# lukemelas/deep-spectral-segmentation

Hardware: AMD Instinct MI355X
Metric: images/sec end-to-end (features+eigs) at 480², K=5; eigvec cos-err vs CPU (higher is better)
Workload: dtype f16

## Files before the change

### deep-spectral-segmentation_amd/csrc/linear384.hip

```cpp
#include "common.h"
#include "kres.h"
#include <type_traits>
#include <utility>

#ifdef DSS_LIN_TIMELINE
__device__ unsigned long long dss_lin_tl[8];
#define DSS_TL_DECL unsigned long long tl_t = __builtin_readcyclecounter(), tl_acc[4] = {0, 0, 0, 0}; const unsigned long long tl_r0 = wall_clock64();
#define DSS_TL_MARK(i) { const unsigned long long n_ = __builtin_readcyclecounter(); tl_acc[i] += n_ - tl_t; tl_t = n_; }
#define DSS_TL_FLUSH if (threadIdx.x == 0) { for (int i_ = 0; i_ < 4; ++i_) atomicAdd(&dss_lin_tl[i_], tl_acc[i_]); atomicAdd(&dss_lin_tl[4], 1ull); atomicAdd(&dss_lin_tl[5], wall_clock64() - tl_r0); }
#else
#define DSS_TL_DECL
#define DSS_TL_MARK(i)
#define DSS_TL_FLUSH
#endif

namespace dss {

static constexpr int LBN = 32;
static constexpr int LGELU_ILP = 2;

template <int OFF, class V> __device__ __forceinline__ void lds_read_b128_at(V& dst, unsigned addr) {
  asm volatile("ds_read_b128 %0, %1 offset:%2" : "=v"(dst) : "v"(addr), "n"(OFF));
}
template <int N, class V> __device__ __forceinline__ void lds_wait_for(V& v) {
  asm volatile("s_waitcnt lgkmcnt(%1)" : "+v"(v) : "n"(N));
}
template <int N> __device__ __forceinline__ void wait_vmcnt() { asm volatile("s_waitcnt vmcnt(%0)" ::"n"(N) : "memory"); }
template <int... I, class F> __device__ __forceinline__ void static_for_impl(std::integer_sequence<int, I...>, F&& f) {
  (f(std::integral_constant<int, I>{}), ...);
}
template <int N, class F> __device__ __forceinline__ void static_for(F&& f) {
  static_for_impl(std::make_integer_sequence<int, N>{}, static_cast<F&&>(f));
}

// ... 5 lines not shown
    if (RES && NUNIT > 2) { pp[1] = n; n += 4; }
    for (int v = 0; v < NUNIT; ++v) {
      if (v == u) {
        int last = px[u];
        if (RES && pp[u >> 1] > last) last = pp[u >> 1];
        return n - (last + 4);
      }
      if (ST) n += 4;
      if (v + NXS < NUNIT) { px[v + NXS] = n; n += 4; }
      if (RES && (v & 1) && (v >> 1) + 2 < NUNIT / 2) { pp[(v >> 1) + 2] = n; n += 4; }
    }
    return 0;
  }
};

template <int KS, int RT, int NW> struct LinCfg {
  static_assert(KS * RT == 48 && KS % NW == 0, "the A operand of a wave is 48 fragments");
  static constexpr int WAVES = NW, THREADS = 64 * NW;
  static constexpr int K = 16 * KS;
  static constexpr int ROWS_WAVE = 32 * RT;
  static constexpr int ROWS = ROWS_WAVE * NW;
  static constexpr int CHUNK_BYTES = LBN * K * 2;
  static constexpr int PATCH_BYTES = ROWS_WAVE * 128;
  static constexpr int MAXN = KS == 24 ? 2048 : 3072;
  static constexpr int NSTORE = 4 * RT;
};

struct KfOut { float* k32; float* rnorm; int Tn; float eps; const unsigned char* img; const float* pos; int H, W, Wp; };

template <class T, int GELU, int KS, int RT, int NW, int LNM, int MODE>
__device__ __forceinline__ void linear_kres_body(const T* __restrict__ A, float* __restrict__ X,
                                                 const T* __restrict__ R, long r_ld, long r_plane, float eps,
                                                 const T* __restrict__ W,
                                                 const T* __restrict__ bias, const float* __restrict__ aux,
                                                 T* __restrict__ C, int M, int N, int planar, const KfOut kf) {
  typedef typename vec8<T>::type V8;
  typedef typename vec4<T>::type V4;
  typedef LinCfg<KS, RT, NW> Cfg;
  constexpr int LK = Cfg::K, LKS = KS, LBM = Cfg::ROWS, LWAVES = NW, LTHREADS = Cfg::THREADS;
  __shared__ __attribute__((aligned(256))) unsigned char Ws[2][Cfg::CHUNK_BYTES];
  __shared__ __attribute__((aligned(256))) unsigned char Stg[LWAVES][Cfg::PATCH_BYTES];
  const int tid = threadIdx.x;
  const int lane = tid & 63, wave = tid >> 6;
  const int li = lane & 31, hh = lane >> 5;
  const int mrem = M - blockIdx.x * LBM;
  const int rloc = wave * Cfg::ROWS_WAVE;
  const bool block_full = mrem >= LBM;

  DSS_TL_DECL
  V8 a[RT][LKS];
  float am[RT];
  if constexpr (MODE == 4) {
    static_assert(RT == 1 && LK == 768, "one 16 x 16 x 3 patch per operand row");
    typedef unsigned u32x2v __attribute__((ext_vector_type(2)));
    const unsigned gp = (unsigned)min((int)blockIdx.x * LBM + rloc + li, M - 1);
    const unsigned pb = gp / (unsigned)kf.Tn, pn = gp - pb * (unsigned)kf.Tn;
    const unsigned py0 = (pn / (unsigned)kf.Wp) * 16u, px0 = (pn - (pn / (unsigned)kf.Wp) * (unsigned)kf.Wp) * 16u;
    const unsigned w3 = (unsigned)kf.W * 3u;
// ... 45 lines not shown
      if constexpr (rd + 1 < NROUND) wait_vmcnt<NPIECE>();
      else wait_vmcnt<0>();
      const unsigned char* pw = pbuf[rd & 1];
#pragma unroll
      for (int t = 0; t < RT; ++t)
#pragma unroll
        for (int sl = 0; sl < 4; ++sl)
          a[t][4 * rd + sl] = *reinterpret_cast<const V8*>(pw + (32 * t + li) * 128 + ((((unsigned)(2 * sl + hh)) ^ fsw) << 4));
      asm volatile("s_waitcnt lgkmcnt(0)" ::: "memory");
      if constexpr (rd + 2 < NROUND) issue_round(rd + 2);
    });
    __syncthreads();
  } else {
    typedef __attribute__((address_space(3))) void* lds3_t;
    typedef float f32x4v __attribute__((ext_vector_type(4)));
    constexpr bool RES = LNM == 2;
    constexpr int NCB = LK / 32, NUNIT = RT * NCB;
    constexpr int WS_SHARE = 2 * Cfg::CHUNK_BYTES / LWAVES;
    constexpr int NSLOT = (WS_SHARE + Cfg::PATCH_BYTES) / 4096;
    constexpr int NXS = RES ? NSLOT - 2 : NSLOT;
    static_assert(WS_SHARE % 4096 == 0 && Cfg::PATCH_BYTES % 4096 == 0 && NXS >= 2 && NCB % 2 == 0 && NUNIT <= 48, "LN prologue layout");
    constexpr bool XST = RES && MODE != 2;
    typedef LnSched<NUNIT, NXS, RES, XST> Sched;
    unsigned char* const ws_share = &Ws[0][0] + wave * WS_SHARE;
    unsigned char* const patch = &Stg[wave][0];
    auto slot_ptr = [&](int i) -> unsigned char* { return i * 4096 < WS_SHARE ? ws_share + i * 4096 : patch + (i * 4096 - WS_SHARE); };
    const size_t row0 = (size_t)blockIdx.x * LBM;
    const unsigned char* const xblk = reinterpret_cast<const unsigned char*>(X) + row0 * (size_t)(LK * 4);
    const unsigned char* const rblk = reinterpret_cast<const unsigned char*>(R) + row0 * (size_t)r_ld * 2;
    const unsigned r_ldb = (unsigned)r_ld * 2u;
    const unsigned fsw16 = 16u * (unsigned)((li >> 1) & 7);
    const int prow = lane >> 3;
    const unsigned pch16[2] = {16u * (unsigned)((lane & 7) ^ (lane >> 4)), 16u * (unsigned)((lane & 7) ^ (4 + (lane >> 4)))};
    auto dma = [&](unsigned lds_addr, unsigned voff, const unsigned char* sbase) {
      unsigned keep;
      asm volatile("s_mov_b32 %0, m0\n\ts_mov_b32 m0, %1\n\ts_nop 0\n\tglobal_load_lds_dwordx4 %2, %3\n\t"
                   "s_mov_b32 m0, %0"
                   : "=&s"(keep) : "s"(lds_addr), "v"(voff), "s"(sbase) : "memory");
// ... 6 lines not shown
    auto rowc = [&](int t, int q) { return (unsigned)min(rloc + 32 * t + 8 * q + prow, mrem - 1); };
    auto issue_x = [&](int u) {
      const int t = u / NCB, cb = u % NCB;
      const unsigned dst = __builtin_amdgcn_readfirstlane((unsigned)(size_t)(lds3_t)slot_ptr(u % NXS));
      const unsigned char* src = uniform_ptr(xblk + 128 * cb);
#pragma unroll
      for (int q = 0; q < 4; ++q) dma(dst + 1024u * q, rowc(t, q) * (unsigned)(LK * 4) + pch16[q & 1], src);
    };
    auto issue_p = [&](int j) {
      const int t = (2 * j) / NCB, g = ((2 * j) % NCB) >> 1;
      const unsigned dst = __builtin_amdgcn_readfirstlane((unsigned)(size_t)(lds3_t)slot_ptr(NXS + (j & 1)));
      const unsigned char* src = uniform_ptr(rblk + (size_t)g * (size_t)r_plane * 2);
#pragma unroll
      for (int q = 0; q < 4; ++q) dma(dst + 1024u * q, rowc(t, q) * r_ldb + pch16[q & 1], src);
    };
    float piv[RT], s1[RT], s2[RT];
#pragma unroll
    for (int t = 0; t < RT; ++t) { piv[t] = 0.f; s1[t] = 0.f; s2[t] = 0.f; }
    if (RES) issue_p(0);
#pragma unroll
    for (int i = 0; i < NXS && i < NUNIT; ++i) issue_x(i);
    if (RES && NUNIT > 2) issue_p(1);
    static_for<NUNIT>([&](auto uc) {
      constexpr int u = decltype(uc)::value;
      constexpr int t = u / NCB, cb = u % NCB, o = cb & 1;
      if (block_full) wait_vmcnt<Sched::after(u)>();
      else wait_vmcnt<0>();
      unsigned char* xs = slot_ptr(u % NXS);
      unsigned char* xr = xs + li * 128;
      f32x4v v0[2], v1[2];
#pragma unroll
      for (int sl = 0; sl < 2; ++sl) {
        v0[sl] = *reinterpret_cast<const f32x4v*>(xr + ((16u * (4 * sl + 2 * hh)) ^ fsw16));
        v1[sl] = *reinterpret_cast<const f32x4v*>(xr + ((16u * (4 * sl + 2 * hh + 1)) ^ fsw16));
      }
      if constexpr (RES) {
        const unsigned char* pr = slot_ptr(NXS + ((u >> 1) & 1)) + li * 128;
#pragma unroll
        for (int sl = 0; sl < 2; ++sl) {
          const V8 pv = *reinterpret_cast<const V8*>(pr + ((16u * (4 * o + 2 * sl + hh)) ^ fsw16));
#pragma unroll
          for (int e = 0; e < 4; ++e) { v0[sl][e] += to_f32<T>(pv[e]); v1[sl][e] += to_f32<T>(pv[4 + e]); }
        }
      }
      if constexpr (cb == 0) {
        const float g0 = __builtin_amdgcn_fmed3f(v0[0][0], v0[0][1], v0[0][2]), g1 = __builtin_amdgcn_fmed3f(v1[0][0], v1[0][1], v1[0][2]);
        const float g2 = __builtin_amdgcn_fmed3f(v0[1][0], v0[1][1], v0[1][2]);
        const unsigned pm = __float_as_uint(__builtin_amdgcn_fmed3f(g0, g1, g2));
        const auto pr = __builtin_amdgcn_permlane32_swap(pm, pm, false, false);
        const unsigned plo = pr[0];
        piv[t] = __uint_as_float(plo);
// ... 20 lines not shown
#pragma unroll
        for (int sl = 0; sl < 2; ++sl) {
          *reinterpret_cast<f32x4v*>(xr + ((16u * (4 * sl + 2 * hh)) ^ fsw16)) = v0[sl];
          *reinterpret_cast<f32x4v*>(xr + ((16u * (4 * sl + 2 * hh + 1)) ^ fsw16)) = v1[sl];
        }
        asm volatile("s_waitcnt lgkmcnt(0)" ::: "memory");
        unsigned char* xw = const_cast<unsigned char*>(xblk) + 128 * cb;
#pragma unroll
        for (int q = 0; q < 4; ++q) {
          const f32x4v lin = *reinterpret_cast<const f32x4v*>(xs + 1024 * q + 16 * lane);
          if (block_full || rloc + 32 * t + 8 * q + prow < mrem)
            *reinterpret_cast<f32x4v*>(xw + rowc(t, q) * (unsigned)(LK * 4) + pch16[q & 1]) = lin;
        }
      }
      asm volatile("s_waitcnt lgkmcnt(0)" ::: "memory");
      if (u + NXS < NUNIT) issue_x(u + NXS);
      if (RES && (u & 1) && (u >> 1) + 2 < NUNIT / 2) issue_p((u >> 1) + 2);
    });
    constexpr float HN = (float)(LK / 2);
#pragma unroll
    for (int t = 0; t < RT; ++t) {
      const float mh = piv[t] + s1[t] * (1.0f / HN), m2h = fmaxf(s2[t] - s1[t] * s1[t] * (1.0f / HN), 0.f);
      const float mo = __shfl_xor(mh, 32, 64), m2o = __shfl_xor(m2h, 32, 64);
      const float mean = 0.5f * (mh + mo), dl = mo - mh;
      const float var = (m2h + m2o + dl * dl * (0.5f * HN)) * (1.0f / (float)LK);
      am[t] = hh ? (var + eps) * rsqrtf(var + eps) : mean - piv[t];
    }
    __syncthreads();
  }

  constexpr int NST = LKS / LWAVES;
  const unsigned gsrc0 = (unsigned)(li * (LK * 2) + 16 * hh + 32 * (wave * NST));
// ... 283 lines not shown
    DSS_TL_MARK(3)
  }
  if constexpr (MODE == 2) kf_finish();
  DSS_TL_FLUSH
}

template <class T, int GELU, int KS, int RT, int NW, int LNM, int MODE = 0>
__global__ __launch_bounds__(64 * NW, NW == 8 ? 1 : 2) void linear_kres_kernel(const T* __restrict__ A, float* __restrict__ X,
                                                                 const T* __restrict__ R, long r_ld, long r_plane, float eps,
                                                                 const T* __restrict__ W,
                                                                 const T* __restrict__ bias, const float* __restrict__ aux,
                                                                 T* __restrict__ C, int M, int N, int planar) {
  linear_kres_body<T, GELU, KS, RT, NW, LNM, MODE>(A, X, R, r_ld, r_plane, eps, W, bias, aux, C, M, N, planar, KfOut{nullptr, nullptr, 0, 0.f, nullptr, nullptr, 0, 0, 0});
}

template <class T>
__global__ __launch_bounds__(512, 1) void patch_embed_kres_kernel(const unsigned char* __restrict__ img, const T* __restrict__ Wp,
                                                                  const T* __restrict__ biasp, const float* __restrict__ pos,
                                                                  float* __restrict__ x, int M, int N, int Np, int H, int W, int Wpat) {
  linear_kres_body<T, 0, 48, 1, 8, 0, 4>(nullptr, nullptr, nullptr, 0, 0, 0.f, Wp, biasp, nullptr, nullptr, M, N, 0,
                                             KfOut{x, nullptr, Np, 0.f, img, pos, H, W, Wpat});
}

template <class T, int KS, int RT, int NW, int LNM>
__global__ __launch_bounds__(64 * NW, NW == 8 ? 1 : 2) void kfeat_kres_kernel(float* __restrict__ X, const T* __restrict__ R, long r_ld, long r_plane, float eps,
                                                            const T* __restrict__ W, const float* __restrict__ aux, f16* __restrict__ k16,
                                                            float* __restrict__ k32, float* __restrict__ rnorm, int M, int Tn, float norm_eps) {
  linear_kres_body<T, 0, KS, RT, NW, LNM, 2>(nullptr, X, R, r_ld, r_plane, eps, W, nullptr, aux, reinterpret_cast<T*>(k16), M, 16 * KS, 0,
                                                 KfOut{k32, rnorm, Tn, norm_eps, nullptr, nullptr, 0, 0, 0});
}
// ... 26 lines not shown
  if constexpr (std::is_same<T, f16>::value) {
    if (gelu == 2) {
      hipLaunchKernelGGL((linear_kres_kernel<T, 2, KS, RT, NW, LNM, MODE>), dim3(blocks), dim3(64 * NW), 0, s, (const T*)A, X,
                         (const T*)R, r_ld, r_plane, eps, (const T*)W, (const T*)bias, aux, (T*)C, M, N, planar);
      return;
    }
  }
  if (gelu)
    hipLaunchKernelGGL((linear_kres_kernel<T, 1, KS, RT, NW, LNM, MODE>), dim3(blocks), dim3(64 * NW), 0, s, (const T*)A, X,
                       (const T*)R, r_ld, r_plane, eps, (const T*)W, (const T*)bias, aux, (T*)C, M, N, planar);
  else
    hipLaunchKernelGGL((linear_kres_kernel<T, 0, KS, RT, NW, LNM, MODE>), dim3(blocks), dim3(64 * NW), 0, s, (const T*)A, X,
                       (const T*)R, r_ld, r_plane, eps, (const T*)W, (const T*)bias, aux, (T*)C, M, N, planar);
}

template <int KS, int RT, int NW>
static int linear_kres(const char* name, const void* A, float* X, const void* res, int res_layout, float eps, const void* W,
                       const void* bias, const float* aux, void* C, int M, int N, int gelu, int out_layout, int dtype,
                       void* stream) {
  typedef LinCfg<KS, RT, NW> Cfg;
  DSS_REQUIRE((A ? bias != nullptr : (X && aux)) && W && C, "%s: null pointer", name);
  DSS_REQUIRE(gelu == 0 || gelu == 1 || (gelu == 2 && dtype == DSS_F16), "%s: gelu must be 0, 1 (fp32 erf form) or 2 (packed-f16 form, DSS_F16 only) (got %d)", name, gelu);
  DSS_REQUIRE(M > 0 && N > 0 && N % (2 * LBN) == 0 && N <= Cfg::MAXN, "%s: need M > 0, N %% %d == 0, N <= %d (M=%d N=%d)",
              name, 2 * LBN, Cfg::MAXN, M, N);
  DSS_REQUIRE(out_layout == DSS_ROW_MAJOR || out_layout == DSS_PLANAR64,
              "%s: out_layout must be DSS_ROW_MAJOR or DSS_PLANAR64 (got %d)", name, out_layout);
  DSS_REQUIRE(A || res_layout == DSS_ROW_MAJOR || res_layout == DSS_PLANAR64,
              "%s: res_layout must be DSS_ROW_MAJOR or DSS_PLANAR64 (got %d)", name, res_layout);
  DSS_REQUIRE(A || (eps >= 0.f && (const void*)X != res && (const void*)X != C && res != C), "%s: eps < 0 or aliased buffers", name);
  hipStream_t s = (hipStream_t)stream;
  const int planar = out_layout == DSS_PLANAR64;
  const long r_ld = res_layout == DSS_PLANAR64 ? 64 : Cfg::K, r_plane = res_layout == DSS_PLANAR64 ? 64L * M : 64;
#define DSS_LAUNCH_KRES(TT)                                                                                              \
  do {                                                                                                                   \
    if (A) launch_linear_kres<TT, KS, RT, NW, 0>(A, nullptr, nullptr, 0, 0, 0.f, W, bias, nullptr, C, M, N, gelu, planar, s); \
    else if (!res) launch_linear_kres<TT, KS, RT, NW, 1>(nullptr, X, nullptr, 0, 0, eps, W, nullptr, aux, C, M, N, gelu, planar, s); \
    else launch_linear_kres<TT, KS, RT, NW, 2>(nullptr, X, res, r_ld, r_plane, eps, W, nullptr, aux, C, M, N, gelu, planar, s); \
  } while (0)
  switch (dtype) {
    case DSS_F16: DSS_LAUNCH_KRES(f16); break;
    case DSS_BF16: DSS_LAUNCH_KRES(bf16); break;
    default: return fail(DSS_ERR_BAD_ARG, "%s: dtype must be DSS_F16 or DSS_BF16 (got %d)", name, dtype);
  }
#undef DSS_LAUNCH_KRES
  DSS_CHECK_LAUNCH(name);
  return DSS_OK;
}

}

extern "C" int dss_linear_k384(const void* A, const void* W, const void* bias, void* C, int M, int N, int gelu,
// ... 19 lines not shown
      hipLaunchKernelGGL((dss::lnlinear_prepare_kernel<dss::f16>), dim3(N), dim3(64), 0, s, W, bias, gamma, beta, (dss::f16*)Wg, aux, K);
      break;
    case DSS_BF16:
      hipLaunchKernelGGL((dss::lnlinear_prepare_kernel<dss::bf16>), dim3(N), dim3(64), 0, s, W, bias, gamma, beta, (dss::bf16*)Wg, aux, K);
      break;
    default: return dss::fail(DSS_ERR_BAD_ARG, "dss_lnlinear_prepare: dtype must be DSS_F16 or DSS_BF16 (got %d)", dtype);
  }
  DSS_CHECK_LAUNCH("dss_lnlinear_prepare");
  return DSS_OK;
}

extern "C" int dss_lnlinear_k384(float* x, const void* residual, int res_layout, float eps, const void* Wg, const float* aux,
                                 void* C, int M, int N, int gelu, int out_layout, int dtype, void* stream) {
  DSS_REQUIRE(x, "dss_lnlinear_k384: null pointer");
  return dss::linear_kres<24, 2, 4>("dss_lnlinear_k384", nullptr, x, residual, res_layout, eps, Wg, nullptr, aux, C, M, N, gelu, out_layout, dtype, stream);
}

extern "C" int dss_patch_embed_p16(const uint8_t* img_u8, const void* Wp, const void* biasp, const float* pos, float* x, int B, int H, int W,
                                   int D, int dtype, void* stream) {
  DSS_REQUIRE(img_u8 && Wp && biasp && pos && x, "dss_patch_embed_p16: null pointer");
  DSS_REQUIRE(B > 0 && H >= 16 && W >= 16, "dss_patch_embed_p16: bad shape B=%d H=%d W=%d", B, H, W);
  typedef dss::LinCfg<48, 1, 8> Cfg;
  DSS_REQUIRE(D > 0 && D % (2 * dss::LBN) == 0 && D <= Cfg::MAXN, "dss_patch_embed_p16: need D %% %d == 0, D <= %d (D=%d)", 2 * dss::LBN, Cfg::MAXN, D);
  const int Hp = H / 16, Wpat = W / 16, Np = Hp * Wpat;
  const long M = (long)B * Np;
  DSS_REQUIRE(M * Np < 4294967296L && (M + B) * D * 4 < 4294967296L && (long)H * W * 3 * B < (1L << 46),
              "dss_patch_embed_p16: B=%d x %d patches exceeds the 32-bit row arithmetic of the epilogue", B, Np);
  const int blocks = dss::ceil_div((int)M, Cfg::ROWS);
  hipStream_t s = (hipStream_t)stream;
  switch (dtype) {
// ... 63 lines not shown
```

### deep-spectral-segmentation_amd/hip.py

```python
from __future__ import annotations

import ctypes
import functools
import os
from ctypes import c_char_p, c_float, c_int, c_size_t, c_uint, c_void_p
from pathlib import Path
from typing import Optional

import torch

PKG = Path(__file__).resolve().parent
LIB_PATH = PKG / "lib" / "libdss_hip.so"

DSS_F32, DSS_F16, DSS_BF16 = 0, 1, 2
_DTYPE_CODE = {torch.float32: DSS_F32, torch.float16: DSS_F16, torch.bfloat16: DSS_BF16}

SYMBOLS = {
    "dss_abi_version": (c_int, []),
    "dss_last_error": (c_char_p, []),
    "dss_target_arch": (c_char_p, []),
    "dss_preprocess_chw": (c_int, [c_void_p, c_void_p, c_int, c_int, c_int, c_void_p]),
    "dss_preprocess_patchify": (c_int, [c_void_p, c_void_p, c_int, c_int, c_int, c_int, c_int, c_void_p]),
    "dss_layernorm_fwd": (c_int, [c_void_p, c_void_p, c_int, c_int, c_void_p, c_void_p, c_void_p, c_int, c_int, c_int,
                                  c_float, c_void_p]),
    "dss_attention_fwd": (c_int, [c_void_p, c_int, c_void_p, c_int, c_int, c_int, c_float, c_int, c_void_p]),
    "dss_linear_k384": (c_int, [c_void_p, c_void_p, c_void_p, c_void_p, c_int, c_int, c_int, c_int, c_int, c_void_p]),
    "dss_linear_k768": (c_int, [c_void_p, c_void_p, c_void_p, c_void_p, c_int, c_int, c_int, c_int, c_int, c_void_p]),
    "dss_linear_lt_workspace_bytes": (c_size_t, []),
    "dss_linear_lt": (c_int, [c_void_p, c_void_p, c_void_p, c_void_p, ctypes.c_long, c_int, c_int, c_int, c_int, c_void_p, c_size_t,
                              c_void_p]),
    "dss_linear_lt_accumulate": (c_int, [c_void_p, c_void_p, c_void_p, c_void_p, ctypes.c_long, c_int, c_int, c_int, c_void_p, c_size_t,
                                         c_void_p]),
    "dss_linear_lt_describe": (c_int, [ctypes.c_long, c_int, c_int, c_int, c_int, c_int, c_size_t, c_char_p, c_size_t]),
    "dss_lnlinear_prepare": (c_int, [c_void_p, c_void_p, c_void_p, c_void_p, c_void_p, c_void_p, c_int, c_int, c_int,
                                     c_void_p]),
    "dss_lnlinear_k384": (c_int, [c_void_p, c_void_p, c_int, c_float, c_void_p, c_void_p, c_void_p, c_int, c_int, c_int,
                                  c_int, c_int, c_void_p]),
    "dss_lnlinear_k768": (c_int, [c_void_p, c_void_p, c_int, c_float, c_void_p, c_void_p, c_void_p, c_int, c_int, c_int,
                                  c_int, c_int, c_void_p]),
    "dss_lnlinear_kfeatures_k384": (c_int, [c_void_p, c_void_p, c_int, c_float, c_void_p, c_void_p, c_void_p, c_void_p,
                                            c_void_p, c_int, c_int, c_float, c_void_p]),
    "dss_lnlinear_kfeatures": (c_int, [c_void_p, c_void_p, c_int, c_float, c_void_p, c_void_p, c_void_p, c_void_p,
                                       c_void_p, c_int, c_int, c_int, c_float, c_int, c_void_p]),
    "dss_patch_embed_p16": (c_int, [c_void_p, c_void_p, c_void_p, c_void_p, c_void_p, c_int, c_int, c_int, c_int, c_int, c_void_p]),
    "dss_normalize_rows": (c_int, [c_void_p, c_void_p, c_int, c_int, c_float, c_void_p]),
    "dss_affinity_ld": (c_int, [c_int]),
    "dss_affinity_elems": (c_size_t, [c_int]),
    "dss_affinity": (c_int, [c_void_p, c_void_p, c_int, c_int, c_int, c_int, c_void_p]),
    "dss_affinity_split_workspace_bytes": (c_size_t, [c_int, c_int, c_int]),
    "dss_affinity_split": (c_int, [c_void_p, c_void_p, c_int, c_int, c_int, c_int, c_float, c_int, c_void_p, c_size_t,
                                   c_void_p]),
    "dss_affinity_split_u16": (c_int, [c_void_p, c_void_p, c_int, c_int, c_int, c_float, c_void_p, c_size_t, c_void_p]),
    "dss_affinity_fused_u16": (c_int, [c_void_p, c_void_p, c_int, c_int, c_int, c_float, c_void_p]),
    "dss_affinity_f16_u16": (c_int, [c_void_p, c_void_p, c_void_p, c_int, c_int, c_int, c_void_p]),
# ... 273 lines not shown

def lnlinear_prepare(weight: torch.Tensor, bias: torch.Tensor, gamma: torch.Tensor, beta: torch.Tensor,
                     dtype: torch.dtype):
    n, k = weight.shape
    for t in (weight, bias, gamma, beta):
        assert t.dtype == torch.float32
    wg = torch.empty((n, k), dtype=dtype, device=weight.device)
    aux = torch.empty((n, 2), dtype=torch.float32, device=weight.device)
    _check(load_library().dss_lnlinear_prepare(_dev(weight, "weight"), _dev(bias, "bias"), _dev(gamma, "gamma"),
                                               _dev(beta, "beta"), _dev(wg, "Wg"), _dev(aux, "aux"), n, k, dtype_code(dtype),
                                               _stream()), "dss_lnlinear_prepare")
    return wg, aux


def lnlinear(x: torch.Tensor, residual: Optional[torch.Tensor], wg: torch.Tensor, aux: torch.Tensor, eps: float,
             gelu: bool = False, planar: bool = False, residual_planar: bool = False) -> torch.Tensor:
    assert x.dtype == torch.float32 and aux.dtype == torch.float32
    k = x.shape[-1]
    if k not in LINEAR_KRES_WIDTHS:
        raise ValueError(f"lnlinear: reduction dimension must be one of {sorted(LINEAR_KRES_WIDTHS)} (got {k})")
    n = wg.shape[0]
    m = x.numel() // k
    assert wg.shape[1] == k and tuple(aux.shape) == (n, 2)
    if residual is not None:
        assert residual.dtype == wg.dtype and tuple(residual.shape) == ((k // 64, m, 64) if residual_planar else tuple(x.shape))
    entry = LINEAR_KRES_WIDTHS[k][0].replace("dss_linear", "dss_lnlinear")
    shape = (n // 64, m, 64) if planar else (*x.shape[:-1], n)
    out = torch.empty(shape, dtype=wg.dtype, device=x.device)
    with _timed("lnlinear", m=m, n=n, k=k, gelu=gelu, res=residual is not None):
        _check(getattr(load_library(), entry)(_dev(x, "x"), 0 if residual is None else _dev(residual, "residual"),
                                              PLANAR64 if residual_planar else ROW_MAJOR, float(eps), _dev(wg, "Wg"),
                                              _dev(aux, "aux"), _dev(out, "out"), m, n, int(gelu),
                                              PLANAR64 if planar else ROW_MAJOR, dtype_code(wg.dtype), _stream()), entry)
    return out


def lnlinear_kfeatures(x: torch.Tensor, residual: Optional[torch.Tensor], wg: torch.Tensor, aux: torch.Tensor, eps: float,
                       norm_eps: float = 1e-12, residual_planar: bool = False, out=None):
    assert x.dtype == torch.float32 and x.dim() == 3 and x.shape[-1] in (384, 768) and x.is_contiguous()
    b, t, d = x.shape
    assert wg.dtype in (torch.float16, torch.bfloat16) and tuple(wg.shape) == (d, d) and tuple(aux.shape) == (d, 2)
    if t <= 64:
        raise ValueError(f"lnlinear_kfeatures: needs more than 64 tokens per image (got {t})")
    if residual is not None:
        assert residual.dtype == wg.dtype and tuple(residual.shape) == ((d // 64, b * t, 64) if residual_planar else (b, t, d))
    if out is not None:
        k32, k16, rn = out
# ... 224 lines not shown
```

### deep-spectral-segmentation_amd/vit.py

```python
from __future__ import annotations

import math
from pathlib import Path
from typing import Dict, Optional, Tuple

import torch
import torch.nn.functional as F

from . import hip
from .synthetic import VIT_CONFIGS

LN_EPS = 1e-6
_TUNING_FILE = Path(__file__).resolve().parent / "tuning" / "tunableop_gfx950.csv"
_gemm_tuning_ready = False


def setup_gemm_tuning(tune_new_shapes: bool = False, use_table: bool = True) -> None:
    global _gemm_tuning_ready
    if not use_table:
        return
    tun = torch.cuda.tunable
    if not _gemm_tuning_ready:
        tun.enable(True)
        if hasattr(tun, "write_file_on_exit"):
# ... 17 lines not shown
    dim = pos_embed.shape[-1]
    side = int(math.sqrt(n0))
    grid = pos_embed[:, 1:].reshape(1, side, side, dim).permute(0, 3, 1, 2)
    grid = F.interpolate(grid, scale_factor=((hp + 0.1) / side, (wp + 0.1) / side), mode="bicubic")
    if (grid.shape[-2], grid.shape[-1]) != (hp, wp):
        raise RuntimeError(f"pos-embed interpolation produced {tuple(grid.shape[-2:])}, wanted {(hp, wp)}")
    grid = grid.permute(0, 2, 3, 1).reshape(1, -1, dim)
    return torch.cat((pos_embed[:, :1], grid), dim=1)


class DinoViT:

    def __init__(self, model_name: str, state_dict: Dict[str, torch.Tensor], device: torch.device,
                 dtype: torch.dtype = torch.float16, k_proj_fp32: bool = False, gelu: str = "auto",
                 linear_kres: int = 2, fuse_ln: bool = True, gemm_tuning: str = "table", fuse_k: bool = True, fuse_pe: bool = True,
                 fuse_qkv768: bool = True, library_gemm: str = "lt", fc2_into_stream: bool = False):
        name = model_name.lower()
        if name not in VIT_CONFIGS:
            raise ValueError(f"Cannot get model: {model_name}")
        if dtype not in (torch.float16, torch.bfloat16):
            raise ValueError("compute dtype must be torch.float16 or torch.bfloat16")
        self.model_name = name
        self.embed_dim, self.depth, self.num_heads, self.patch_size = VIT_CONFIGS[name]
        self.device, self.dtype = torch.device(device), dtype
        self.k_proj_fp32 = k_proj_fp32
        if gelu not in ("auto", "erf", "erf_f16", "tanh_fused"):
            raise ValueError("gelu must be 'auto', 'erf' (DINO's exact GELU, fp32 arithmetic), 'erf_f16' (the same function evaluated on "
                             "packed f16: f16 operands and the K-resident fc1 kernel only) or 'tanh_fused'")
        if gelu == "auto":
            gelu = "erf_f16" if self.embed_dim == 384 else "erf"
        if gelu == "erf_f16" and (dtype != torch.float16 or linear_kres < 2 or self.embed_dim not in hip.LINEAR_KRES_WIDTHS):
            gelu = "erf"
        self.gelu = gelu
        self._gelu_code = 2 if gelu == "erf_f16" else 1
        if linear_kres not in (0, 1, 2):
            raise ValueError("linear_kres must be 0, 1 or 2")
        self.linear_k384 = int(linear_kres)
        self.fuse_ln = bool(fuse_ln)
        self.fuse_k = bool(fuse_k)
        self.fuse_qkv768 = bool(fuse_qkv768)
        if library_gemm not in ("lt", "torch"):
            raise ValueError("library_gemm must be 'lt' (dss_linear_lt) or 'torch' (F.linear)")
        self.library_gemm = library_gemm
        self.fc2_into_stream = bool(fc2_into_stream) and library_gemm == "lt"
        d = self.embed_dim
        sd = state_dict
        need = ["cls_token", "pos_embed", "patch_embed.proj.weight", "patch_embed.proj.bias"]
        for i in range(self.depth):
            for s in ("norm1.weight", "norm1.bias", "attn.qkv.weight", "attn.qkv.bias", "attn.proj.weight",
                      "attn.proj.bias", "norm2.weight", "norm2.bias", "mlp.fc1.weight", "mlp.fc1.bias",
                      "mlp.fc2.weight", "mlp.fc2.bias"):
                need.append(f"blocks.{i}.{s}")
        missing = [k for k in need if k not in sd]
        if missing:
            raise KeyError(f"state_dict is missing {len(missing)} DINO ViT keys, e.g. {missing[:3]}")

        def lp(t):
            return t.detach().to(self.device, dtype).contiguous()

        def f32(t):
# ... 55 lines not shown
        k384 = bool(self.linear_k384) and d == 384
        kres_fc1 = self.gelu in ("erf", "erf_f16") and self.linear_k384 >= 2 and d in hip.LINEAR_KRES_WIDTHS
        lib = ("library GEMM (hipBLASLt through dss_linear_lt: no Stream-K split, verified)" if self.library_gemm == "lt"
               else "library GEMM (hipBLASLt through F.linear)")
        return {
            "patch_embed": "dss_patch_embed_p16 (transform + GEMM + position rows, one kernel)" if self.pe16 is not None
                           else f"dss_preprocess_patchify + {lib} + add",
            "norm1+qkv": f"dss_lnlinear_k{d}" if ("qkv_wg" in blk and self.linear_k384) else
                         ("dss_layernorm_fwd + dss_linear_k384" if k384 else f"dss_layernorm_fwd + {lib}"),
            "attention": "dss_attention_fwd",
            "proj": "dss_linear_k384" if k384 else lib,
            "norm2+fc1+gelu": f"dss_lnlinear_k{d}" if (kres_fc1 and "fc1_wg" in blk) else
                              (f"dss_layernorm_fwd + dss_linear_k{d}" if kres_fc1 else f"dss_layernorm_fwd + {lib} + GELU pass"),
            "gelu": {"erf": "exact-erf form in fp32 (A&S 7.1.28, |err| <= 3e-7)", "erf_f16": "erf-GELU polynomial form on packed f16 (csrc/kres.h)",
                     "tanh_fused": "hipBLASLt's tanh epilogue (NOT the reference function)"}[self.gelu],
            "fc2": lib + (" adding into the fp32 residual stream (dss_linear_lt_accumulate)" if self.fc2_into_stream else ""),
            "hooked norm1 + K projection + hand-over": "dss_lnlinear_kfeatures" if "k_wg" in self.blocks[-1] else
                                                       f"dss_layernorm_fwd + {lib} + dss_kfeatures_finalize",
        }

    def _pos(self, h: int, w: int) -> Tuple[torch.Tensor, torch.Tensor]:
        key = (h, w)
        if key not in self._pos_cache:
            pe = interpolate_pos_encoding(self.pos_embed, self.patch_size, h, w)
            cls_row = (self.cls_token[0, 0] + pe[0, 0]).to(self.device)
            self._pos_cache[key] = (cls_row.contiguous(), pe[0, 1:].to(self.device).contiguous())
        return self._pos_cache[key]

    @torch.no_grad()
    def _run_blocks(self, img_u8: torch.Tensor, nblocks: int):
# ... 8 lines not shown
            key = ("pe16", hp * p, wp * p)
            if key not in self._pos_cache:
                self._pos_cache[key] = (pos + self.pe16[1]).contiguous()
            hip.patch_embed16(img_u8.contiguous(), self.pe16[0], None, self._pos_cache[key], x)
        else:
            patches = hip.preprocess_patchify(img_u8.contiguous(), p, self.dtype)
            tok = self._linear(patches, self.pe_w, self.pe_b, "patch_embed")
            torch.add(tok, pos, out=x[:, 1:])

        pending = None
        k384 = self.linear_k384 and d == 384
        kres_fc1 = self.gelu in ("erf", "erf_f16") and self.linear_k384 >= 2 and d in hip.LINEAR_KRES_WIDTHS
        for i in range(nblocks):
            blk = self.blocks[i]
            qkv_planar = bool(k384)
            if "qkv_wg" in blk and self.linear_k384:
                qkv = hip.lnlinear(x, pending, blk["qkv_wg"], blk["qkv_aux"], LN_EPS, planar=True)
                qkv_planar = True
            else:
                hcur = hip.layernorm(x, blk["n1w"], blk["n1b"], LN_EPS, self.dtype, residual=pending)
                if k384:
                    qkv = hip.linear_kres(hcur, blk["qkv_w"], blk["qkv_b"], planar=True)
                else:
                    qkv = self._linear(hcur, blk["qkv_w"], blk["qkv_b"], "qkv")
            o = hip.attention(qkv, heads, self.scale, planar_bt=(b, t)) if qkv_planar else hip.attention(qkv, heads, self.scale)
            if k384:
                pending = hip.linear_kres(o, blk["proj_w"], blk["proj_b"], planar=True)
            else:
                pending = self._linear(o, blk["proj_w"], blk["proj_b"], "proj")
            if kres_fc1 and "fc1_wg" in blk:
                f1 = hip.lnlinear(x, pending, blk["fc1_wg"], blk["fc1_aux"], LN_EPS, gelu=self._gelu_code, residual_planar=bool(k384))
            else:
                hcur = hip.layernorm(x, blk["n2w"], blk["n2b"], LN_EPS, self.dtype, residual=pending,
                                     residual_planar=bool(k384))
                if kres_fc1:
                    f1 = hip.linear_kres(hcur, blk["fc1_w"], blk["fc1_b"], gelu=self._gelu_code)
                elif self.gelu in ("erf", "erf_f16"):
                    f1 = F.gelu(self._linear(hcur, blk["fc1_w"], blk["fc1_b"], "fc1"))
                else:
                    f1 = torch._addmm_activation(blk["fc1_b"], hcur.view(b * t, d), blk["fc1_w"].t(),
                                                 use_gelu=True).view(b, t, -1)
            if self.fc2_into_stream:
                hip.linear_lt_accumulate(f1, blk["fc2_w"], blk["fc2_b32"], x, what="fc2")
                pending = None
            else:
# ... 76 lines not shown
```

### include/dss_hip.h

```cpp
#ifndef DSS_HIP_H
#define DSS_HIP_H

#include <stddef.h>
#include <stdint.h>

#ifdef __cplusplus
extern "C" {
#endif

#define DSS_ABI_VERSION 10

enum { DSS_F32 = 0, DSS_F16 = 1, DSS_BF16 = 2 };

enum { DSS_ROW_MAJOR = 0, DSS_PLANAR64 = 1 };

enum {
  DSS_OK = 0,
  DSS_ERR_BAD_ARG = -1,
  DSS_ERR_HIP = -2,
  DSS_ERR_WORKSPACE = -3,
  DSS_ERR_NO_CONVERGENCE = -4
};

int dss_abi_version(void);
// ... 18 lines not shown

size_t dss_linear_lt_workspace_bytes(void);
int dss_linear_lt(const void* A, const void* W, const void* bias, void* C, long M, int N, int K, int dtype, int out_dtype,
                  void* workspace, size_t workspace_bytes, void* stream);
int dss_linear_lt_describe(long M, int N, int K, int dtype, int out_dtype, int has_bias, size_t workspace_bytes, char* buf,
                           size_t buflen);
int dss_linear_lt_accumulate(const void* A, const void* W, const float* bias, float* X, long M, int N, int K, int dtype,
                             void* workspace, size_t workspace_bytes, void* stream);

int dss_lnlinear_prepare(const float* W, const float* bias, const float* gamma, const float* beta, void* Wg, float* aux,
                         int N, int K, int dtype, void* stream);
int dss_lnlinear_k384(float* x, const void* residual, int res_layout, float eps, const void* Wg, const float* aux, void* C,
                      int M, int N, int gelu, int out_layout, int dtype, void* stream);
int dss_lnlinear_k768(float* x, const void* residual, int res_layout, float eps, const void* Wg, const float* aux, void* C,
                      int M, int N, int gelu, int out_layout, int dtype, void* stream);

int dss_lnlinear_kfeatures_k384(float* x, const void* residual, int res_layout, float eps, const void* Wg, const float* aux,
                                float* k32, void* k16, float* rnorm, int M, int T, float norm_eps, void* stream);
int dss_lnlinear_kfeatures(float* x, const void* residual, int res_layout, float eps, const void* Wg, const float* aux,
                           float* k32, void* k16, float* rnorm, int M, int T, int D, float norm_eps, int dtype, void* stream);

int dss_patch_embed_p16(const uint8_t* img_u8, const void* Wp, const void* biasp, const float* pos, float* x, int B, int H, int W,
                        int D, int dtype, void* stream);

int dss_normalize_rows(const float* x, float* y, int rows, int D, float eps, void* stream);

int dss_affinity_ld(int N);
size_t dss_affinity_elems(int N);
int dss_affinity(const float* feats, float* W, int B, int N, int D, int threshold_at_zero,
                 void* stream);
// ... 40 lines not shown
```

Measured before the change: 13860.

## Store the fp32 residual stream once per ViT block via read-only and two-residual LN-Linear

Adds a read-only LN+Linear variant for the qkv path, which normalises x plus the pending residual without writing the sum back. It also adds a two-residual variant for fc1 that adds the previous fc2 output and the attention projection output in its prologue and stores the updated stream once. The goal is to cut one fp32 read-modify-write of the residual stream per block. In exchange the fc1 prologue loads an extra f16 residual tile through a new DMA schedule, which adds LDS slot pressure and a new schedule helper.

```diff
diff --git a/deep-spectral-segmentation_amd/csrc/linear384.hip b/deep-spectral-segmentation_amd/csrc/linear384.hip
--- a/deep-spectral-segmentation_amd/csrc/linear384.hip
+++ b/deep-spectral-segmentation_amd/csrc/linear384.hip
@@ -18,6 +18,7 @@
 
 static constexpr int LBN = 32;
 static constexpr int LGELU_ILP = 2;
+static constexpr int LN2_RD = 2;
 
 template <int OFF, class V> __device__ __forceinline__ void lds_read_b128_at(V& dst, unsigned addr) {
   asm volatile("ds_read_b128 %0, %1 offset:%2" : "=v"(dst) : "v"(addr), "n"(OFF));
@@ -53,6 +54,23 @@
   }
 };
 
+template <int NUNIT, int NXS, int RD> struct LnSched2 {
+  static constexpr int after(int u) {
+    int n = 0, px[64] = {}, pp[64] = {};
+    for (int i = 0; i < NUNIT && i < (NXS > RD ? NXS : RD); ++i) {
+      if (i < RD) { n += 4; pp[i] = n; }
+      if (i < NXS) { n += 4; px[i] = n; }
+    }
+    for (int v = 0; v < NUNIT; ++v) {
+      if (v == u) return n - (px[u] > pp[u] ? px[u] : pp[u]);
+      n += 4;
+      if (v + RD < NUNIT) { n += 4; pp[v + RD] = n; }
+      if (v + NXS < NUNIT) { n += 4; px[v + NXS] = n; }
+    }
+    return 0;
+  }
+};
+
 template <int KS, int RT, int NW> struct LinCfg {
   static_assert(KS * RT == 48 && KS % NW == 0, "the A operand of a wave is 48 fragments");
   static constexpr int WAVES = NW, THREADS = 64 * NW;
@@ -72,7 +90,8 @@
                                                  const T* __restrict__ R, long r_ld, long r_plane, float eps,
                                                  const T* __restrict__ W,
                                                  const T* __restrict__ bias, const float* __restrict__ aux,
-                                                 T* __restrict__ C, int M, int N, int planar, const KfOut kf) {
+                                                 T* __restrict__ C, int M, int N, int planar, const KfOut kf,
+                                                 const T* __restrict__ R2 = nullptr, long r2_ld = 0, long r2_plane = 0) {
   typedef typename vec8<T>::type V8;
   typedef typename vec4<T>::type V4;
   typedef LinCfg<KS, RT, NW> Cfg;
@@ -80,7 +99,7 @@
   __shared__ __attribute__((aligned(256))) unsigned char Ws[2][Cfg::CHUNK_BYTES];
   __shared__ __attribute__((aligned(256))) unsigned char Stg[LWAVES][Cfg::PATCH_BYTES];
   const int tid = threadIdx.x;
-  const int lane = tid & 63, wave = tid >> 6;
+  const int lane = tid & 63, wave = LNM == 4 ? __builtin_amdgcn_readfirstlane(tid >> 6) : tid >> 6;
   const int li = lane & 31, hh = lane >> 5;
   const int mrem = M - blockIdx.x * LBM;
   const int rloc = wave * Cfg::ROWS_WAVE;
@@ -156,14 +175,16 @@
   } else {
     typedef __attribute__((address_space(3))) void* lds3_t;
     typedef float f32x4v __attribute__((ext_vector_type(4)));
-    constexpr bool RES = LNM == 2;
+    constexpr bool RES = LNM >= 2, RES2 = LNM == 4;
+    static_assert(LNM <= 2 || (KS == 24 && MODE == 0), "the read-only and two-residual prologues are built for the K = 384 Linear mode only");
     constexpr int NCB = LK / 32, NUNIT = RT * NCB;
     constexpr int WS_SHARE = 2 * Cfg::CHUNK_BYTES / LWAVES;
     constexpr int NSLOT = (WS_SHARE + Cfg::PATCH_BYTES) / 4096;
-    constexpr int NXS = RES ? NSLOT - 2 : NSLOT;
+    constexpr int RD2 = LN2_RD;
+    constexpr int NXS = RES2 ? NSLOT - RD2 : RES ? NSLOT - 2 : NSLOT;
     static_assert(WS_SHARE % 4096 == 0 && Cfg::PATCH_BYTES % 4096 == 0 && NXS >= 2 && NCB % 2 == 0 && NUNIT <= 48, "LN prologue layout");
-    constexpr bool XST = RES && MODE != 2;
-    typedef LnSched<NUNIT, NXS, RES, XST> Sched;
+    constexpr bool XST = RES && MODE != 2 && LNM != 3;
+    typedef std::conditional_t<RES2, LnSched2<NUNIT, NXS, RD2>, LnSched<NUNIT, NXS, RES, XST>> Sched;
     unsigned char* const ws_share = &Ws[0][0] + wave * WS_SHARE;
     unsigned char* const patch = &Stg[wave][0];
     auto slot_ptr = [&](int i) -> unsigned char* { return i * 4096 < WS_SHARE ? ws_share + i * 4096 : patch + (i * 4096 - WS_SHARE); };
@@ -200,13 +221,41 @@
 #pragma unroll
       for (int q = 0; q < 4; ++q) dma(dst + 1024u * q, rowc(t, q) * r_ldb + pch16[q & 1], src);
     };
+    auto rtile_ptr = [&](int s, int u) -> unsigned char* {
+      const int o = NXS * 4096 + 2048 * (s * RD2 + u % RD2);
+      return o < WS_SHARE ? ws_share + o : patch + (o - WS_SHARE);
+    };
+    auto issue_p2 = [&](int u) {
+      const int t = u / NCB, cb = u % NCB;
+      unsigned fl;
+      asm volatile("v_mbcnt_lo_u32_b32 %0, -1, 0\n\tv_mbcnt_hi_u32_b32 %0, -1, %0" : "=v"(fl));
+      const unsigned ch16 = 16u * ((fl & 3u) ^ ((fl >> 4) & 3u));
+#pragma unroll
+      for (int s = 0; s < 2; ++s) {
+        const unsigned dst = __builtin_amdgcn_readfirstlane((unsigned)(size_t)(lds3_t)rtile_ptr(s, u));
+        const unsigned char* blk2 = s ? reinterpret_cast<const unsigned char*>(R2) + row0 * (size_t)r2_ld * 2 : rblk;
+        const unsigned char* src = uniform_ptr(blk2 + (size_t)(cb >> 1) * (size_t)(s ? r2_plane : r_plane) * 2 + 64 * (cb & 1));
+        const unsigned ldb = s ? (unsigned)r2_ld * 2u : r_ldb;
+#pragma unroll
+        for (int q = 0; q < 2; ++q)
+          dma(dst + 1024u * q, (unsigned)min(rloc + 32 * t + 16 * q + (int)(fl >> 2), mrem - 1) * ldb + ch16, src);
+      }
+    };
     float piv[RT], s1[RT], s2[RT];
 #pragma unroll
     for (int t = 0; t < RT; ++t) { piv[t] = 0.f; s1[t] = 0.f; s2[t] = 0.f; }
-    if (RES) issue_p(0);
-#pragma unroll
-    for (int i = 0; i < NXS && i < NUNIT; ++i) issue_x(i);
-    if (RES && NUNIT > 2) issue_p(1);
+    if constexpr (RES2) {
+#pragma unroll
+      for (int i = 0; i < NUNIT && i < (NXS > RD2 ? NXS : RD2); ++i) {
+        if (i < RD2) issue_p2(i);
+        if (i < NXS) issue_x(i);
+      }
+    } else {
+      if (RES) issue_p(0);
+#pragma unroll
+      for (int i = 0; i < NXS && i < NUNIT; ++i) issue_x(i);
+      if (RES && NUNIT > 2) issue_p(1);
+    }
     static_for<NUNIT>([&](auto uc) {
       constexpr int u = decltype(uc)::value;
       constexpr int t = u / NCB, cb = u % NCB, o = cb & 1;
@@ -220,7 +269,19 @@
         v0[sl] = *reinterpret_cast<const f32x4v*>(xr + ((16u * (4 * sl + 2 * hh)) ^ fsw16));
         v1[sl] = *reinterpret_cast<const f32x4v*>(xr + ((16u * (4 * sl + 2 * hh + 1)) ^ fsw16));
       }
-      if constexpr (RES) {
+      if constexpr (RES2) {
+        const unsigned rsw16 = 16u * (unsigned)((li >> 2) & 3);
+#pragma unroll
+        for (int s = 0; s < 2; ++s) {
+          const unsigned char* pr = rtile_ptr(s, u) + li * 64;
+#pragma unroll
+          for (int sl = 0; sl < 2; ++sl) {
+            const V8 pv = *reinterpret_cast<const V8*>(pr + ((16u * (2 * sl + hh)) ^ rsw16));
+#pragma unroll
+            for (int e = 0; e < 4; ++e) { v0[sl][e] += to_f32<T>(pv[e]); v1[sl][e] += to_f32<T>(pv[4 + e]); }
+          }
+        }
+      } else if constexpr (RES) {
         const unsigned char* pr = slot_ptr(NXS + ((u >> 1) & 1)) + li * 128;
 #pragma unroll
         for (int sl = 0; sl < 2; ++sl) {
@@ -271,8 +332,13 @@
         }
       }
       asm volatile("s_waitcnt lgkmcnt(0)" ::: "memory");
-      if (u + NXS < NUNIT) issue_x(u + NXS);
-      if (RES && (u & 1) && (u >> 1) + 2 < NUNIT / 2) issue_p((u >> 1) + 2);
+      if constexpr (RES2) {
+        if (u + RD2 < NUNIT) issue_p2(u + RD2);
+        if (u + NXS < NUNIT) issue_x(u + NXS);
+      } else {
+        if (u + NXS < NUNIT) issue_x(u + NXS);
+        if (RES && (u & 1) && (u >> 1) + 2 < NUNIT / 2) issue_p((u >> 1) + 2);
+      }
     });
     constexpr float HN = (float)(LK / 2);
 #pragma unroll
@@ -586,6 +652,15 @@
   linear_kres_body<T, GELU, KS, RT, NW, LNM, MODE>(A, X, R, r_ld, r_plane, eps, W, bias, aux, C, M, N, planar, KfOut{nullptr, nullptr, 0, 0.f, nullptr, nullptr, 0, 0, 0});
 }
 
+template <class T, int GELU>
+__global__ __launch_bounds__(256, 2) void linear_kres2_kernel(float* __restrict__ X, const T* __restrict__ R, long r_ld, long r_plane,
+                                                              const T* __restrict__ R2, long r2_ld, long r2_plane, float eps,
+                                                              const T* __restrict__ W, const float* __restrict__ aux, T* __restrict__ C,
+                                                              int M, int N, int planar) {
+  linear_kres_body<T, GELU, 24, 2, 4, 4, 0>(nullptr, X, R, r_ld, r_plane, eps, W, nullptr, aux, C, M, N, planar,
+                                            KfOut{nullptr, nullptr, 0, 0.f, nullptr, nullptr, 0, 0, 0}, R2, r2_ld, r2_plane);
+}
+
 template <class T>
 __global__ __launch_bounds__(512, 1) void patch_embed_kres_kernel(const unsigned char* __restrict__ img, const T* __restrict__ Wp,
                                                                   const T* __restrict__ biasp, const float* __restrict__ pos,
@@ -642,11 +717,29 @@
                        (const T*)R, r_ld, r_plane, eps, (const T*)W, (const T*)bias, aux, (T*)C, M, N, planar);
 }
 
+template <class T>
+static void launch_linear_kres2(float* X, const void* R, long r_ld, long r_plane, const void* R2, long r2_ld, long r2_plane, float eps,
+                                const void* W, const float* aux, void* C, int M, int N, int gelu, int planar, hipStream_t s) {
+  const int blocks = ceil_div(M, LinCfg<24, 2, 4>::ROWS);
+#define DSS_LAUNCH_KRES2(G)                                                                                                      \
+  hipLaunchKernelGGL((linear_kres2_kernel<T, G>), dim3(blocks), dim3(256), 0, s, X, (const T*)R, r_ld, r_plane, (const T*)R2, r2_ld, \
+                     r2_plane, eps, (const T*)W, aux, (T*)C, M, N, planar)
+  if constexpr (std::is_same<T, f16>::value) {
+    if (gelu == 2) { DSS_LAUNCH_KRES2(2); return; }
+  }
+  if (gelu) DSS_LAUNCH_KRES2(1);
+  else DSS_LAUNCH_KRES2(0);
+#undef DSS_LAUNCH_KRES2
+}
+
 template <int KS, int RT, int NW>
 static int linear_kres(const char* name, const void* A, float* X, const void* res, int res_layout, float eps, const void* W,
                        const void* bias, const float* aux, void* C, int M, int N, int gelu, int out_layout, int dtype,
-                       void* stream) {
+                       void* stream, bool store = true, const void* res2 = nullptr, int res2_layout = DSS_ROW_MAJOR) {
   typedef LinCfg<KS, RT, NW> Cfg;
+  DSS_REQUIRE((store && !res2) || (KS == 24 && !A && res && (store || !res2)), "%s: the read-only and two-residual forms need K = 384 and a residual", name);
+  DSS_REQUIRE(!res2 || ((res2_layout == DSS_ROW_MAJOR || res2_layout == DSS_PLANAR64) && res2 != (const void*)X && res2 != C),
+              "%s: res2_layout must be DSS_ROW_MAJOR or DSS_PLANAR64 (got %d) and residual2 must not alias x or C", name, res2_layout);
   DSS_REQUIRE((A ? bias != nullptr : (X && aux)) && W && C, "%s: null pointer", name);
   DSS_REQUIRE(gelu == 0 || gelu == 1 || (gelu == 2 && dtype == DSS_F16), "%s: gelu must be 0, 1 (fp32 erf form) or 2 (packed-f16 form, DSS_F16 only) (got %d)", name, gelu);
   DSS_REQUIRE(M > 0 && N > 0 && N % (2 * LBN) == 0 && N <= Cfg::MAXN, "%s: need M > 0, N %% %d == 0, N <= %d (M=%d N=%d)",
@@ -659,10 +752,13 @@
   hipStream_t s = (hipStream_t)stream;
   const int planar = out_layout == DSS_PLANAR64;
   const long r_ld = res_layout == DSS_PLANAR64 ? 64 : Cfg::K, r_plane = res_layout == DSS_PLANAR64 ? 64L * M : 64;
+  const long r2_ld = res2_layout == DSS_PLANAR64 ? 64 : Cfg::K, r2_plane = res2_layout == DSS_PLANAR64 ? 64L * M : 64;
 #define DSS_LAUNCH_KRES(TT)                                                                                              \
   do {                                                                                                                   \
     if (A) launch_linear_kres<TT, KS, RT, NW, 0>(A, nullptr, nullptr, 0, 0, 0.f, W, bias, nullptr, C, M, N, gelu, planar, s); \
     else if (!res) launch_linear_kres<TT, KS, RT, NW, 1>(nullptr, X, nullptr, 0, 0, eps, W, nullptr, aux, C, M, N, gelu, planar, s); \
+    else if (KS == 24 && res2) launch_linear_kres2<TT>(X, res, r_ld, r_plane, res2, r2_ld, r2_plane, eps, W, aux, C, M, N, gelu, planar, s); \
+    else if (KS == 24 && !store) launch_linear_kres<TT, 24, 2, 4, 3>(nullptr, X, res, r_ld, r_plane, eps, W, nullptr, aux, C, M, N, gelu, planar, s); \
     else launch_linear_kres<TT, KS, RT, NW, 2>(nullptr, X, res, r_ld, r_plane, eps, W, nullptr, aux, C, M, N, gelu, planar, s); \
   } while (0)
   switch (dtype) {
@@ -712,6 +808,21 @@
                                  void* C, int M, int N, int gelu, int out_layout, int dtype, void* stream) {
   DSS_REQUIRE(x, "dss_lnlinear_k384: null pointer");
   return dss::linear_kres<24, 2, 4>("dss_lnlinear_k384", nullptr, x, residual, res_layout, eps, Wg, nullptr, aux, C, M, N, gelu, out_layout, dtype, stream);
+}
+
+extern "C" int dss_lnlinear_ro_k384(const float* x, const void* residual, int res_layout, float eps, const void* Wg, const float* aux,
+                                    void* C, int M, int N, int gelu, int out_layout, int dtype, void* stream) {
+  DSS_REQUIRE(x && residual, "dss_lnlinear_ro_k384: null pointer (x and residual are required)");
+  return dss::linear_kres<24, 2, 4>("dss_lnlinear_ro_k384", nullptr, const_cast<float*>(x), residual, res_layout, eps, Wg, nullptr, aux, C, M, N, gelu,
+                                    out_layout, dtype, stream, false);
+}
+
+extern "C" int dss_lnlinear_res2_k384(float* x, const void* residual, int res_layout, const void* residual2, int res2_layout, float eps,
+                                      const void* Wg, const float* aux, void* C, int M, int N, int gelu, int out_layout, int dtype,
+                                      void* stream) {
+  DSS_REQUIRE(x && residual && residual2, "dss_lnlinear_res2_k384: null pointer (x and both residuals are required)");
+  return dss::linear_kres<24, 2, 4>("dss_lnlinear_res2_k384", nullptr, x, residual, res_layout, eps, Wg, nullptr, aux, C, M, N, gelu, out_layout,
+                                    dtype, stream, true, residual2, res2_layout);
 }
 
 extern "C" int dss_patch_embed_p16(const uint8_t* img_u8, const void* Wp, const void* biasp, const float* pos, float* x, int B, int H, int W,
diff --git a/deep-spectral-segmentation_amd/hip.py b/deep-spectral-segmentation_amd/hip.py
--- a/deep-spectral-segmentation_amd/hip.py
+++ b/deep-spectral-segmentation_amd/hip.py
@@ -38,6 +38,10 @@
                                   c_int, c_int, c_void_p]),
     "dss_lnlinear_k768": (c_int, [c_void_p, c_void_p, c_int, c_float, c_void_p, c_void_p, c_void_p, c_int, c_int, c_int,
                                   c_int, c_int, c_void_p]),
+    "dss_lnlinear_ro_k384": (c_int, [c_void_p, c_void_p, c_int, c_float, c_void_p, c_void_p, c_void_p, c_int, c_int, c_int,
+                                     c_int, c_int, c_void_p]),
+    "dss_lnlinear_res2_k384": (c_int, [c_void_p, c_void_p, c_int, c_void_p, c_int, c_float, c_void_p, c_void_p, c_void_p, c_int,
+                                       c_int, c_int, c_int, c_int, c_void_p]),
     "dss_lnlinear_kfeatures_k384": (c_int, [c_void_p, c_void_p, c_int, c_float, c_void_p, c_void_p, c_void_p, c_void_p,
                                             c_void_p, c_int, c_int, c_float, c_void_p]),
     "dss_lnlinear_kfeatures": (c_int, [c_void_p, c_void_p, c_int, c_float, c_void_p, c_void_p, c_void_p, c_void_p,
@@ -341,7 +345,8 @@
 
 
 def lnlinear(x: torch.Tensor, residual: Optional[torch.Tensor], wg: torch.Tensor, aux: torch.Tensor, eps: float,
-             gelu: bool = False, planar: bool = False, residual_planar: bool = False) -> torch.Tensor:
+             gelu: bool = False, planar: bool = False, residual_planar: bool = False, store: bool = True,
+             residual2: Optional[torch.Tensor] = None, residual2_planar: bool = False) -> torch.Tensor:
     assert x.dtype == torch.float32 and aux.dtype == torch.float32
     k = x.shape[-1]
     if k not in LINEAR_KRES_WIDTHS:
@@ -349,15 +354,25 @@
     n = wg.shape[0]
     m = x.numel() // k
     assert wg.shape[1] == k and tuple(aux.shape) == (n, 2)
+    if not store or residual2 is not None:
+        if k != 384:
+            raise ValueError(f"lnlinear: store=False and residual2 exist for K = 384 only (got {k})")
+        if residual is None or (not store and residual2 is not None):
+            raise ValueError("lnlinear: store=False needs `residual` and no `residual2`; `residual2` needs `residual`")
     if residual is not None:
         assert residual.dtype == wg.dtype and tuple(residual.shape) == ((k // 64, m, 64) if residual_planar else tuple(x.shape))
+    if residual2 is not None:
+        assert residual2.dtype == wg.dtype and tuple(residual2.shape) == ((k // 64, m, 64) if residual2_planar else tuple(x.shape))
     entry = LINEAR_KRES_WIDTHS[k][0].replace("dss_linear", "dss_lnlinear")
     shape = (n // 64, m, 64) if planar else (*x.shape[:-1], n)
     out = torch.empty(shape, dtype=wg.dtype, device=x.device)
+    head = [_dev(x, "x"), 0 if residual is None else _dev(residual, "residual"), PLANAR64 if residual_planar else ROW_MAJOR]
+    if residual2 is not None:
+        entry, head = "dss_lnlinear_res2_k384", head + [_dev(residual2, "residual2"), PLANAR64 if residual2_planar else ROW_MAJOR]
+    elif not store:
+        entry = "dss_lnlinear_ro_k384"
     with _timed("lnlinear", m=m, n=n, k=k, gelu=gelu, res=residual is not None):
-        _check(getattr(load_library(), entry)(_dev(x, "x"), 0 if residual is None else _dev(residual, "residual"),
-                                              PLANAR64 if residual_planar else ROW_MAJOR, float(eps), _dev(wg, "Wg"),
-                                              _dev(aux, "aux"), _dev(out, "out"), m, n, int(gelu),
+        _check(getattr(load_library(), entry)(*head, float(eps), _dev(wg, "Wg"), _dev(aux, "aux"), _dev(out, "out"), m, n, int(gelu),
                                               PLANAR64 if planar else ROW_MAJOR, dtype_code(wg.dtype), _stream()), entry)
     return out
 
diff --git a/deep-spectral-segmentation_amd/vit.py b/deep-spectral-segmentation_amd/vit.py
--- a/deep-spectral-segmentation_amd/vit.py
+++ b/deep-spectral-segmentation_amd/vit.py
@@ -55,7 +55,7 @@
     def __init__(self, model_name: str, state_dict: Dict[str, torch.Tensor], device: torch.device,
                  dtype: torch.dtype = torch.float16, k_proj_fp32: bool = False, gelu: str = "auto",
                  linear_kres: int = 2, fuse_ln: bool = True, gemm_tuning: str = "table", fuse_k: bool = True, fuse_pe: bool = True,
-                 fuse_qkv768: bool = True, library_gemm: str = "lt", fc2_into_stream: bool = False):
+                 fuse_qkv768: bool = True, library_gemm: str = "lt", fc2_into_stream: bool = False, stream_store: str = "auto"):
         name = model_name.lower()
         if name not in VIT_CONFIGS:
             raise ValueError(f"Cannot get model: {model_name}")
@@ -84,7 +84,11 @@
             raise ValueError("library_gemm must be 'lt' (dss_linear_lt) or 'torch' (F.linear)")
         self.library_gemm = library_gemm
         self.fc2_into_stream = bool(fc2_into_stream) and library_gemm == "lt"
+        if stream_store not in ("auto", "twice"):
+            raise ValueError("stream_store must be 'auto' or 'twice'")
         d = self.embed_dim
+        self.stream_once = (stream_store == "auto" and d == 384 and self.fuse_ln and self.linear_k384 >= 2
+                            and self.gelu in ("erf", "erf_f16") and not self.fc2_into_stream)
         sd = state_dict
         need = ["cls_token", "pos_embed", "patch_embed.proj.weight", "patch_embed.proj.bias"]
         for i in range(self.depth):
@@ -170,6 +174,10 @@
                               (f"dss_layernorm_fwd + dss_linear_k{d}" if kres_fc1 else f"dss_layernorm_fwd + {lib} + GELU pass"),
             "gelu": {"erf": "exact-erf form in fp32 (A&S 7.1.28, |err| <= 3e-7)", "erf_f16": "erf-GELU polynomial form on packed f16 (csrc/kres.h)",
                      "tanh_fused": "hipBLASLt's tanh epilogue (NOT the reference function)"}[self.gelu],
+            "residual stream": ("stored once per block (dss_lnlinear_ro_k384 + dss_lnlinear_res2_k384 behind block 0)" if self.stream_once
+                                else "stored twice per block (by each fused norm -> Linear kernel)" if ("qkv_wg" in blk and kres_fc1 and "fc1_wg" in blk
+                                                                                                       and not self.fc2_into_stream)
+                                else "as the norm / fc2 path of this model stores it"),
             "fc2": lib + (" adding into the fp32 residual stream (dss_linear_lt_accumulate)" if self.fc2_into_stream else ""),
             "hooked norm1 + K projection + hand-over": "dss_lnlinear_kfeatures" if "k_wg" in self.blocks[-1] else
                                                        f"dss_layernorm_fwd + {lib} + dss_kfeatures_finalize",
@@ -208,8 +216,10 @@
         for i in range(nblocks):
             blk = self.blocks[i]
             qkv_planar = bool(k384)
+            once = self.stream_once and pending is not None
+            prev = pending
             if "qkv_wg" in blk and self.linear_k384:
-                qkv = hip.lnlinear(x, pending, blk["qkv_wg"], blk["qkv_aux"], LN_EPS, planar=True)
+                qkv = hip.lnlinear(x, pending, blk["qkv_wg"], blk["qkv_aux"], LN_EPS, planar=True, store=not once)
                 qkv_planar = True
             else:
                 hcur = hip.layernorm(x, blk["n1w"], blk["n1b"], LN_EPS, self.dtype, residual=pending)
@@ -222,7 +232,9 @@
                 pending = hip.linear_kres(o, blk["proj_w"], blk["proj_b"], planar=True)
             else:
                 pending = self._linear(o, blk["proj_w"], blk["proj_b"], "proj")
-            if kres_fc1 and "fc1_wg" in blk:
+            if once:
+                f1 = hip.lnlinear(x, prev, blk["fc1_wg"], blk["fc1_aux"], LN_EPS, gelu=self._gelu_code, residual2=pending, residual2_planar=True)
+            elif kres_fc1 and "fc1_wg" in blk:
                 f1 = hip.lnlinear(x, pending, blk["fc1_wg"], blk["fc1_aux"], LN_EPS, gelu=self._gelu_code, residual_planar=bool(k384))
             else:
                 hcur = hip.layernorm(x, blk["n2w"], blk["n2b"], LN_EPS, self.dtype, residual=pending,
diff --git a/include/dss_hip.h b/include/dss_hip.h
--- a/include/dss_hip.h
+++ b/include/dss_hip.h
@@ -56,6 +56,10 @@
                       int M, int N, int gelu, int out_layout, int dtype, void* stream);
 int dss_lnlinear_k768(float* x, const void* residual, int res_layout, float eps, const void* Wg, const float* aux, void* C,
                       int M, int N, int gelu, int out_layout, int dtype, void* stream);
+int dss_lnlinear_ro_k384(const float* x, const void* residual, int res_layout, float eps, const void* Wg, const float* aux, void* C,
+                         int M, int N, int gelu, int out_layout, int dtype, void* stream);
+int dss_lnlinear_res2_k384(float* x, const void* residual, int res_layout, const void* residual2, int res2_layout, float eps,
+                           const void* Wg, const float* aux, void* C, int M, int N, int gelu, int out_layout, int dtype, void* stream);
 
 int dss_lnlinear_kfeatures_k384(float* x, const void* residual, int res_layout, float eps, const void* Wg, const float* aux,
                                 float* k32, void* k16, float* rnorm, int M, int T, float norm_eps, void* stream);
```

Result: no change. 14000, median of 6 (+1.0%).
